# cruiseresearchgroup/ViLCo

Measured on AMD Instinct MI355X. Metric: clips/sec (fwd+bwd) MQ transformer T=2304 C=2304, higher is better.
Workload: dtype fp16 MFMA on 2-part splits of power-of-two scaled fp32 operands (22 significant bits, 3 MFMAs per product), fp32 accumulate: fp32-equivalent; weight-gradient products with contraction length >= 2048 use the leading fp16 parts only (11-bit operands, 1 MFMA; <= 3.5e-4 of the 3-MFMA gradients at this c; 1 GPU; MQ ViLCo backbone config P: T=2304 Cin=2304 D=1024 H=16 arch(2,2,5) XLNet layer text L=77x768 22 classes, train mode with the reference's dropout 0.1 / droppath 0.1 / XLNet dropout 0.1 (mq_vilco.yaml, xlnet_config_1024.json); clips_per_gpu=2, global_batch=2, parallelism=dp1

## Files before the change

include/vilco_hip.h:

```cpp
#ifndef VILCO_HIP_H
#define VILCO_HIP_H

#include <stddef.h>
#include <stdint.h>

#ifdef __cplusplus
extern "C" {
#endif

enum vilco_status {
  VILCO_OK = 0,
  VILCO_ERR_BADARG = -1,
  VILCO_ERR_UNSUPPORTED = -2,
  VILCO_ERR_LAUNCH = -3,
  VILCO_ERR_WORKSPACE = -4
};

const char* vilco_status_str(int status);
const char* vilco_version(void);
size_t vilco_abi_sizeof(const char* struct_name);

enum { VILCO_ACT_NONE = 0, VILCO_ACT_RELU = 1, VILCO_ACT_GELU = 2 };
enum { VILCO_TAP_NONE = 0, VILCO_TAP_A = 1, VILCO_TAP_B = 2 };

typedef struct vilco_gemm_desc {
  const float* A;
  const float* B;
  float* C;
  int32_t M, N, K;
  int32_t a_kcontig;
  int32_t b_kcontig;
  int64_t lda, ldb, ldc;
  int32_t batch_outer, batch_inner;
  int64_t sAo, sAi, sBo, sBi, sCo, sCi;
  int32_t tap_operand, tapC, tapT;
  int32_t precision;
  float alpha, beta;
  const float* bias;
  float* preact;
  int32_t act;
  const int32_t* row_len;
  int32_t rowT;
  const float* colscale;
  const float* residual;
  int32_t res_masked;
  void* workspace;
  size_t workspace_bytes;
  const void* a_planes;
  const void* b_planes;
  int32_t band, bandT;
  float drop_p;
  uint32_t drop_seed;
  float* amax_out;
  const float* a_amax; int32_t a_namax;
  const float* b_amax; int32_t b_namax;
  int32_t a_planes_seq, b_planes_seq;
  const float* row_mask;
} vilco_gemm_desc;

size_t vilco_gemm_workspace(const vilco_gemm_desc* d);
int vilco_gemm(const vilco_gemm_desc* d, void* stream);
int vilco_gemm_group(const vilco_gemm_desc* descs, int32_t n, void* stream);
size_t vilco_gemm_group_workspace(const vilco_gemm_desc* d, int32_t n);
int vilco_gemm_set_group_dw(int32_t on);
int32_t vilco_gemm_group_dw(void);

int vilco_gemm_force(int32_t bm, int32_t ks);
int vilco_gemm_set_skinny(int32_t on);
int64_t vilco_gemm_config_gen(void);
int32_t vilco_gemm_amax_parts(const vilco_gemm_desc* desc);
int vilco_gemm_profile_begin(void);
int vilco_gemm_profile_end(double* kernel_ms, int64_t* launches);
int64_t vilco_gemm_profile_records(int64_t* desc, double* ms, int64_t cap);

size_t vilco_pack_bytes(int64_t rows, int64_t cols, int32_t precision);
int vilco_pack(const float* src, int64_t rows, int64_t cols, int64_t ld, int32_t precision, void* planes,
               size_t planes_bytes, void* stream);
typedef struct vilco_pack_item {
  const float* src;
  int64_t rows, cols, ld;
  void* planes;
  size_t planes_bytes;
  int32_t nbatch;
  int64_t batch_stride;
  int32_t relshift;
  const float* amax;
  int32_t namax;
  int32_t seq_len;
} vilco_pack_item;
size_t vilco_pack_item_bytes(const vilco_pack_item* item, int32_t precision);
int vilco_pack_many(const vilco_pack_item* items, int32_t n, int32_t precision, void* stream);

typedef struct vilco_ln_fwd_desc {
  const float* x;
  const float* gamma;
  const float* beta;
  float* y;
  float* mean;
  float* rstd;
  int64_t rows;
  int32_t C;
  float eps;
  int32_t relu;
  float* amax_parts;
  int32_t* n_parts;
  void* planes;
  size_t planes_bytes;
  int32_t seq_len;
  const float* row_mask;
  int64_t mask_rows;
} vilco_ln_fwd_desc;
size_t vilco_layernorm_planes_bytes(int64_t rows, int32_t C, int32_t seq_len);
int vilco_layernorm_fwd(const vilco_ln_fwd_desc* d, void* stream);

typedef struct vilco_ln_bwd_desc {
// ... 441 lines not shown
```

vilco_amd/_lib.py:

```python
import ctypes as C
import os

_HERE = os.path.dirname(os.path.abspath(__file__))
if __package__:
    from . import switches
else:
    import importlib.util
    _spec = importlib.util.spec_from_file_location("vilco_switches", os.path.join(_HERE, "switches.py"))
    switches = importlib.util.module_from_spec(_spec)
    _spec.loader.exec_module(switches)
LIB_PATH = switches.text("VILCO_HIP_LIB") or os.path.join(_HERE, "libvilco_hip.so")

ACT_NONE, ACT_RELU, ACT_GELU = 0, 1, 2
TAP_NONE, TAP_A, TAP_B = 0, 1, 2

c_fp = C.c_void_p
i32, i64, f32, sz = C.c_int32, C.c_int64, C.c_float, C.c_size_t


class GemmDesc(C.Structure):
    _cname_ = "vilco_gemm_desc"
    _fields_ = [
        ("A", c_fp), ("B", c_fp), ("C", c_fp),
        ("M", i32), ("N", i32), ("K", i32),
# ... 109 lines not shown


class DistillDesc(C.Structure):
    _cname_ = "vilco_distill_desc"
    _fields_ = [("logits", c_fp), ("targets", c_fp), ("level_row", c_fp), ("level_T", c_fp), ("level_dev", c_fp),
                ("B", i32), ("R", i32), ("C", i32), ("L", i32), ("clip", i32), ("ldt", i32), ("n_known", i32), ("mode", i32),
                ("scale", f32)]


class DerDesc(C.Structure):
    _cname_ = "vilco_der_desc"
    _fields_ = [("logits", c_fp), ("level_row", c_fp), ("level_T", c_fp), ("level_dev", c_fp), ("level_len", c_fp),
                ("der_tab", c_fp), ("B", i32), ("R", i32), ("C", i32), ("L", i32), ("alpha", C.c_double)]


class PodDesc(C.Structure):
    _cname_ = "vilco_pod_desc"
    _fields_ = [("feats", c_fp), ("level_T", c_fp), ("level_len", c_fp), ("pod_tab", c_fp), ("B", i32), ("C", i32), ("L", i32),
                ("reserved", i32), ("scale", C.c_double)]


class BicCorrectDesc(C.Structure):
    _cname_ = "vilco_bic_correct_desc"
    _fields_ = [("x", c_fp), ("y", c_fp), ("splits", c_fp), ("table", c_fp), ("rows", i64), ("C", i32), ("S", i32),
                ("ldx", i32), ("ldy", i32), ("n_layers", i32)]


class PromptDesc(C.Structure):
    _cname_ = "vilco_prompt_desc"
    _fields_ = [("x", c_fp), ("prompt", c_fp), ("key", c_fp), ("cls", c_fp), ("idx_in", c_fp),
                ("B", i32), ("L", i32), ("C", i32), ("P", i32), ("len", i32), ("k", i32), ("key_mode", i32), ("vote", i32),
                ("idx", c_fp), ("sim", c_fp), ("pn", c_fp), ("xn", c_fp), ("selkey", c_fp), ("prompted", c_fp),
                ("reduce_sim", c_fp), ("workspace", c_fp), ("workspace_bytes", sz)]


class CodaDesc(C.Structure):
    _cname_ = "vilco_coda_desc"
    _fields_ = [("x", c_fp), ("prompt", c_fp), ("key", c_fp), ("attn", c_fp),
                ("B", i32), ("L", i32), ("C", i32), ("M", i32), ("len", i32), ("s", i32), ("f", i32), ("want_ortho", i32),
                ("alpha", c_fp), ("prompted", c_fp), ("ortho", c_fp), ("workspace", c_fp), ("workspace_bytes", sz)]


SIGNATURES = {
    "vilco_status_str": (C.c_char_p, [C.c_int]),
    "vilco_version": (C.c_char_p, []),
    "vilco_abi_sizeof": (sz, [C.c_char_p]),
    "vilco_defer_set": (C.c_int, [i32]),
    "vilco_defer_pending": (i64, []),
    "vilco_defer_flush": (C.c_int, [c_fp]),
    "vilco_gemm_workspace": (sz, [C.POINTER(GemmDesc)]),
    "vilco_gemm": (C.c_int, [C.POINTER(GemmDesc), c_fp]),
    "vilco_gemm_group": (C.c_int, [C.POINTER(GemmDesc), i32, c_fp]),
    "vilco_gemm_group_workspace": (sz, [C.POINTER(GemmDesc), i32]),
    "vilco_gemm_set_group_dw": (C.c_int, [i32]),
    "vilco_gemm_group_dw": (i32, []),
    "vilco_gemm_amax_parts": (i32, [C.POINTER(GemmDesc)]),
    "vilco_gemm_force": (C.c_int, [i32, i32]),
    "vilco_gemm_set_skinny": (C.c_int, [i32]),
    "vilco_gemm_config_gen": (i64, []),
    "vilco_gemm_profile_begin": (C.c_int, []),
    "vilco_gemm_profile_end": (C.c_int, [C.POINTER(C.c_double), C.POINTER(C.c_int64)]),
    "vilco_gemm_profile_records": (C.c_int64, [C.POINTER(C.c_int64), C.POINTER(C.c_double), C.c_int64]),
    "vilco_pack_bytes": (sz, [i64, i64, i32]),
    "vilco_pack_item_bytes": (sz, [C.POINTER(PackItem), i32]),
    "vilco_pack": (C.c_int, [c_fp, i64, i64, i64, i32, c_fp, sz, c_fp]),
    "vilco_pack_many": (C.c_int, [C.POINTER(PackItem), i32, i32, c_fp]),
    "vilco_layernorm_fwd": (C.c_int, [C.POINTER(LnFwdDesc), c_fp]),
    "vilco_layernorm_planes_bytes": (sz, [i64, i32, i32]),
    "vilco_layernorm_bwd_workspace": (sz, [i64, i32]),
    "vilco_layernorm_bwd": (C.c_int, [C.POINTER(LnBwdDesc), c_fp]),
    "vilco_dwconv3_fwd": (C.c_int, [c_fp, c_fp, c_fp, c_fp, i32, i32, i32, i32, c_fp]),
    "vilco_dwconv3_bwd_workspace": (sz, [i32, i32, i32, i32]),
    "vilco_dwconv3_bwd": (C.c_int, [c_fp, c_fp, c_fp, c_fp, c_fp, c_fp, i32, i32, i32, i32, c_fp, sz, c_fp]),
    "vilco_maxpool3s2_fwd": (C.c_int, [c_fp, c_fp, c_fp, i32, i32, i32, c_fp]),
    "vilco_maxpool3s2_bwd": (C.c_int, [c_fp, c_fp, c_fp, c_fp, i32, i32, i32, c_fp]),
    "vilco_softmax_fwd": (C.c_int, [c_fp, c_fp, i32, i32, i32, i32, i32, c_fp]),
    "vilco_softmax_bwd": (C.c_int, [c_fp, c_fp, i32, i32, i32, i32, c_fp]),
    "vilco_relshift_add": (C.c_int, [c_fp, c_fp, f32, i32, i32, i32, c_fp]),
    "vilco_relshift_bwd": (C.c_int, [c_fp, c_fp, f32, i32, i32, i32, c_fp]),
    "vilco_attn_supported": (C.c_int, [i32]),
    "vilco_attn_fwd_workspace": (sz, [i32, i32, i32, i32, i32, i32]),
    "vilco_attn_amax_parts": (i32, [i32, i32, i32, i32, i32, i32, i32, f32, i32]),
    "vilco_attn_fwd": (C.c_int, [C.POINTER(AttnDesc), c_fp]),
    "vilco_attn_planes_supported": (i32, [i32, i32, i32, i32, i32, i32, f32]),
    "vilco_attn_bwd_workspace": (sz, [i32, i32, i32, i32, i32, i32]),
    "vilco_attn_bwd": (C.c_int, [C.POINTER(AttnDesc), c_fp]),
    "vilco_attn_dsplanes_bytes": (sz, [i32, i32, i32]),
    "vilco_xl_scores_workspace": (sz, [i32, i32, i32, i32]),
    "vilco_xl_scores": (C.c_int, [c_fp, c_fp, c_fp, i32, i32, i32, i32, i32, i32, c_fp, sz, c_fp]),
    "vilco_decode_workspace": (sz, [i32, i32]),
    "vilco_decode": (C.c_int, [c_fp, c_fp, c_fp, c_fp, c_fp, i32, i32, i32, f32, f32, c_fp, c_fp, c_fp, c_fp, c_fp, sz, c_fp]),
    "vilco_scale_add_fwd": (C.c_int, [c_fp, c_fp, c_fp, c_fp, c_fp, c_fp, i32, i32, i32, i32, c_fp]),
    "vilco_colsum_workspace": (sz, [i64, i32]),
    "vilco_scale_add_bwd": (C.c_int, [C.POINTER(ScaleAddBwdDesc), c_fp]),
    "vilco_dropout": (C.c_int, [c_fp, c_fp, i64, f32, C.c_uint32, C.c_uint64, c_fp]),
    "vilco_attn_dropout_mask": (C.c_int, [c_fp, i64, i32, f32, C.c_uint32, c_fp]),
    "vilco_seed_word_set": (C.c_int, [C.c_uint32, c_fp]),
    "vilco_seed_word_bump": (C.c_int, [c_fp]),
    "vilco_seed_word_get": (C.c_int, [C.POINTER(C.c_uint32)]),
    "vilco_axpby": (C.c_int, [c_fp, c_fp, c_fp, f32, f32, i64, c_fp]),
    "vilco_act_bwd": (C.c_int, [C.POINTER(ActBwdDesc), c_fp]),
    "vilco_act_bwd_planes_bytes": (sz, [i64, i32, i32]),
    "vilco_colsum": (C.c_int, [c_fp, c_fp, i64, i32, c_fp, sz, c_fp]),
    "vilco_mask_rows": (C.c_int, [c_fp, c_fp, i32, i32, i32, c_fp]),
    "vilco_add_pe": (C.c_int, [c_fp, c_fp, c_fp, c_fp, i32, i32, i32, c_fp]),
    "vilco_transpose2d": (C.c_int, [c_fp, c_fp, i32, i32, i32, c_fp]),
# ... 112 lines not shown
```

vilco_amd/csrc/gemm.hip:

```cpp
#include <algorithm>
#include <climits>
#include <cstdlib>
#include <type_traits>
#include <utility>
#include <vector>
#include "common.h"
#include "pack.h"

namespace {

constexpr int BN = 128, BK = 32;
constexpr int EPI_LD = 68;

__device__ __forceinline__ int swz(int row) { return (4 - ((row >> 2) & 3)) & 3; }
__device__ __forceinline__ int lds_off(int row, int chunk) { return row * 32 + ((chunk ^ swz(row)) << 3); }

struct Epi {
  float alpha, beta;
  const float* bias;
  float* preact;
  int act;
  const int* row_len;
  int rowT;
  const float* colscale;
// ... 802 lines not shown
#pragma unroll
          for (int j = 0; j < 4; ++j) acc[i][j] = mma<true>(fa[u][0][i], fb[u][1][j], acc[i][j]);
#pragma unroll
        for (int i = 0; i < MB; ++i)
#pragma unroll
          for (int j = 0; j < 4; ++j) acc[i][j] = mma<true>(fa[u][1][i], fb[u][0][j], acc[i][j]);
      }
    }
  }

  float* mine = part + wave * (BMS * SK_LD);
#pragma unroll
  for (int i = 0; i < MB; ++i)
#pragma unroll
    for (int j = 0; j < 4; ++j)
#pragma unroll
      for (int rr = 0; rr < 4; ++rr) mine[(16 * i + (lane >> 4) * 4 + rr) * SK_LD + 16 * j + r16] = acc[i][j][rr];
  __syncthreads();
  const float inv = g.inv_a[0] * g.inv_b[0];
  float am = 0.f;
#pragma unroll 1
  for (int q = tid; q < BMS * 16; q += 512) {
    const int row = q >> 4, c4 = (q & 15) * 4;
    const float* src = part + row * SK_LD + c4;
    f32x4 v = *reinterpret_cast<const f32x4*>(src);
#pragma unroll
    for (int w = 1; w < 8; ++w) v += *reinterpret_cast<const f32x4*>(src + w * (BMS * SK_LD));
    v *= inv;
    const int m = m0 + row, n = n0 + c4;
    if (m >= g.M || n >= g.N) continue;
    const long idx = (long)m * g.ldc + n;
    bool valid = g.e.row_len ? (m % g.e.rowT) < g.e.row_len[m / g.e.rowT] : true;
    if (g.e.row_mask) valid = valid && g.e.row_mask[m] != 0.f;
    if (g.vec_out) am = fmaxf(am, store_out4(g, idx, n, v, valid));
    else
#pragma unroll 1
      for (int e = 0; e < 4; ++e) if (n + e < g.N) am = fmaxf(am, store_out(g, idx + e, n + e, v[e], valid));
  }
  if (g.amax_out) {
    am = wave_max(am);
    __syncthreads();
    if (lane == 0) part[wave] = am;
    __syncthreads();
    if (tid == 0) {
      float m = part[0];
#pragma unroll
      for (int w = 1; w < 8; ++w) m = fmaxf(m, part[w]);
      g.amax_out[blockIdx.x] = m;
    }
  }
}

template <bool VEC>
__global__ __launch_bounds__(256) void splitk_reduce_kernel(GArgs g, int nz) {
  constexpr int V = VEC ? 4 : 1;
  const int NV = g.N / V;
  const long per = (long)g.M * NV;
  const long total = per * nz;
  float am = 0.f;
  for (long i = (long)blockIdx.x * blockDim.x + threadIdx.x; i < total; i += (long)gridDim.x * blockDim.x) {
    const int z = (int)(i / per);
    const long mn = i % per;
    const int m = (int)(mn / NV), n = (int)(mn % NV) * V;
    const int zo = z / g.batch_inner, zi = z % g.batch_inner;
    const long idx = zo * g.sCo + zi * g.sCi + (long)m * g.ldc + n;
    bool valid = true;
    if (g.e.row_len) valid = (m % g.e.rowT) < g.e.row_len[m / g.e.rowT];
    if (g.e.row_mask) valid = valid && g.e.row_mask[m] != 0.f;
    if (VEC) {
      f32x4 s = {0.f, 0.f, 0.f, 0.f};
      int k = 0;
      for (; k + 4 <= g.ksplit; k += 4) {
        f32x4 v[4];
#pragma unroll
        for (int u = 0; u < 4; ++u) v[u] = *reinterpret_cast<const f32x4*>(g.c + (long)(k + u) * g.split_stride + idx);
#pragma unroll
        for (int u = 0; u < 4; ++u) s += v[u];
      }
      if (k + 2 <= g.ksplit) {
        const f32x4 v0 = *reinterpret_cast<const f32x4*>(g.c + (long)k * g.split_stride + idx);
        const f32x4 v1 = *reinterpret_cast<const f32x4*>(g.c + (long)(k + 1) * g.split_stride + idx);
        s += v0; s += v1;
        k += 2;
      }
      if (k < g.ksplit) s += *reinterpret_cast<const f32x4*>(g.c + (long)k * g.split_stride + idx);
      am = fmaxf(am, store_out4(g, idx, n, s, valid));
    } else {
      float s = 0.f;
      for (int k = 0; k < g.ksplit; ++k) s += g.c[(long)k * g.split_stride + idx];
      am = fmaxf(am, store_out(g, idx, n, s, valid));
    }
  }
  if (g.amax_out) {
    __shared__ float red[4];
    am = wave_max(am);
    if ((threadIdx.x & 63) == 0) red[threadIdx.x >> 6] = am;
    __syncthreads();
    if (threadIdx.x == 0) g.amax_out[blockIdx.x] = fmaxf(fmaxf(red[0], red[1]), fmaxf(red[2], red[3]));
  }
}

inline long align_up(long x, long a) { return (x + a - 1) / a * a; }
constexpr long SCALE_BYTES = 2 * AMAX_MAX_BLOCKS * 4 + 256;
constexpr long PACK_HDR = VILCO_PACK_HDR;

struct Config {
  const bool km = vilco_env_int("VILCO_GEMM_KM", 1, INT_MIN) != 0;
  const bool k2 = vilco_env_flag("VILCO_GEMM_K2", true);
  const bool sub192 = vilco_env_flag("VILCO_GEMM_SUB192", true);
  const bool dw_tall = vilco_env_flag("VILCO_GEMM_DW_TALL", true);
  const bool tapkm = vilco_env_flag("VILCO_CONV_DW_KM", true);
  const bool group = vilco_env_flag("VILCO_GEMM_GROUP", true);
  const int skinny_max_rows = vilco_env_int("VILCO_GEMM_SKINNY_M", 640, 1);
  const int skinny_bm16_rows = vilco_env_int("VILCO_GEMM_SKINNY_BM16", 640, 0);
  const int skinny_max_k = vilco_env_int("VILCO_GEMM_SKINNY_K", 768, 1);
  bool skinny = vilco_env_flag("VILCO_GEMM_SKINNY", true);
  bool group_dw = vilco_env_flag("VILCO_GEMM_GROUP_DW", true);
  int force_bm = vilco_env_int("VILCO_GEMM_BM", 0, INT_MIN), force_ks = vilco_env_int("VILCO_GEMM_KS", 0, INT_MIN);
};
inline Config& config() { static Config c; return c; }
inline int parts_of_precision(int precision, bool pack_abi = false) {
  if (precision == 1) return 1;
  if (precision == 0 || precision == 3) return 2;
  return (precision == 4 && !pack_abi) ? 2 : 3;
}

inline long natural_image_elems(long rows, long cols) { return align_up(rows, 32) * align_up(cols, 32); }
inline long seq_image_elems(long nseq, long T, long cols) { return align_up(vilco_tap_plane_rows(nseq, T) * cols, 8); }

struct Side {
  bool tr, km;
  int tap, out_rows;
  int nbo, nbi;
  long pack_batch;
  long bytes;
  long batch, plane;
};
struct Layout { int NP, Kp; bool tapkm; Side a, b; };

bool tapkm_layout(const vilco_gemm_desc* d, Layout& L) {
  if (!(config().km && config().tapkm && (d->tapC % 8) == 0 && (d->M % 8) == 0 && d->tapT > 0 && (d->K % d->tapT) == 0 &&
        d->batch_outer == 1 && d->batch_inner == 1))
    return false;
  Side &a = L.a, &b = L.b;
  const long nseq = d->K / d->tapT;
  L.Kp = (int)align_up(nseq * (d->tapT + 2) - 1, 32);
  a.tap = b.tap = 1; a.tr = b.tr = false; a.km = b.km = true;
  a.out_rows = L.Kp + 1 + 32; b.out_rows = L.Kp + 3 + 32;
  a.pack_batch = (long)a.out_rows * d->M; b.pack_batch = (long)b.out_rows * d->tapC;
  return true;
}
long prepacked_a(const vilco_gemm_desc* d, const Layout& L) {
  if (L.a.tap != 1) return natural_image_elems(d->M, L.Kp);
  return L.tapkm ? seq_image_elems(d->K / d->tapT, d->tapT, d->M) : seq_image_elems(d->M / d->tapT, d->tapT, d->tapC);
}
long prepacked_b(const vilco_gemm_desc* d, const Layout& L) {
  return L.tapkm ? seq_image_elems(d->K / d->tapT, d->tapT, d->tapC) : natural_image_elems(d->N, L.Kp);
}
void finish_side(const vilco_gemm_desc* d, int NP, Side& s, long so, long si, long image) {
  s.nbo = (so && d->batch_outer > 1) ? d->batch_outer : 1;
  s.nbi = (si && d->batch_inner > 1) ? d->batch_inner : 1;
  s.pack_batch = align_up(s.pack_batch, 8);
  s.bytes = align_up(s.pack_batch * s.nbo * s.nbi * NP * 2, 256);
  s.batch = image >= 0 ? image : s.pack_batch;
  s.plane = s.batch * s.nbo * s.nbi;
}
Layout operand_layout(const vilco_gemm_desc* d, bool a_prepacked, bool b_prepacked) {
  Layout L;
// ... 489 lines not shown
    if (it.planes_bytes < vilco_pack_item_bytes(&it, precision)) return VILCO_ERR_WORKSPACE;
    const long cols = item_cols(it);
    const long rows32 = align_up(it.rows, 32), cols32 = align_up(cols, 32);
    float* hdr = reinterpret_cast<float*>(it.planes);
    PackArgs& pa = pk.a[i];
    pa.src = it.src; pa.dst = reinterpret_cast<__bf16*>(reinterpret_cast<unsigned char*>(it.planes) + PACK_HDR);
    pa.ld = it.ld; pa.rows = (int)it.rows; pa.K = (int)cols; pa.Kp = (int)cols32;
    pa.plane_stride = rows32 * cols32 * nbatch; pa.batch_stride = rows32 * cols32; pa.nbi = nbatch;
    pa.so = 0; pa.si = nbatch > 1 ? it.batch_stride : 0;
    pa.tap = it.relshift ? 4 : 0; pa.tapC = it.relshift ? (int)it.cols : 1; pa.tapT = 1; pa.out_rows = (int)rows32;
    pa.vec = vilco_aligned(it.src, 16) && (it.ld % 4) == 0 && (it.batch_stride % 4) == 0;
    if (it.seq_len > 0) {
      if (it.relshift || nbatch != 1 || (it.cols % 8) != 0 || (it.rows % it.seq_len) != 0) return VILCO_ERR_UNSUPPORTED;
      const long tr = vilco_tap_plane_rows(it.rows / it.seq_len, it.seq_len);
      pa.tap = 1; pa.tapC = (int)it.cols; pa.tapT = it.seq_len; pa.out_rows = (int)tr;
      pa.plane_stride = align_up(tr * it.cols, 8); pa.batch_stride = pa.plane_stride;
    }
    pa.amax = nullptr; pa.namax = 0; pa.inv_scale = hdr + AMAX_MAX_BLOCKS;
    if (precision == 3) {
      PackArgs src_view = pa;
      src_view.K = (int)it.cols; src_view.tap = 0;
      am.op[i] = amax_view(src_view, false, 1, hdr);
      pa.amax = hdr; pa.namax = am.op[i].nblocks;
      if (it.amax && it.namax > 0) { pa.amax = it.amax; pa.namax = it.namax; have_amax[i] = true; }
    }
  }
  if (precision == 3) {
    int todo = 0;
    for (int i = 0; i < n; ++i) todo += have_amax[i] ? 0 : 1;
    if (todo) {
      AmaxArgs am2;
      int k = 0;
      for (int i = 0; i < n; ++i)
        if (!have_amax[i]) am2.op[k++] = am.op[i];
      launch_amax(am2, k, s);
    }
  }
  if (n == 1 && nbatch == 1) dispatch_pack(NP, pk.a[0], false, 1, s);
  else dispatch_pack_multi(NP, pk, n, s, nbatch);
  return vilco_launch_status();
}

extern "C" int vilco_pack(const float* src, int64_t rows, int64_t cols, int64_t ld, int32_t precision, void* planes,
                          size_t planes_bytes, void* stream) {
  const vilco_pack_item it = {src, rows, cols, ld, planes, planes_bytes, 1, 0, 0, nullptr, 0};
  return vilco_pack_many(&it, 1, precision, stream);
}

extern "C" size_t vilco_gemm_workspace(const vilco_gemm_desc* d) {
  if (!d || d->M <= 0 || d->N <= 0 || d->K < 0) return 512;
  return workspace_need(make_plan(d));
}

static void splitk_finish(const vilco_gemm_desc* d, const Prepared& pr) {
  const GArgs& g = pr.g;
  if (vilco_defer_active() && pr.nz == 1 && d->alpha == 1.f && d->beta == 0.f && !d->bias &&
      !d->preact && d->act == VILCO_ACT_NONE && !d->row_len && !d->row_mask && !d->colscale && !d->residual && d->drop_p == 0.f &&
      !d->amax_out) {
    vilco_defer_push_sk(g.c, g.cfinal, g.split_stride, g.ldc, d->M, d->N, pr.p.ksplit);
    return;
  }
  const dim3 blocks((int)splitk_blocks(d));
  if (g.vec_out) hipLaunchKernelGGL(splitk_reduce_kernel<true>, blocks, dim3(256), 0, pr.s, g, pr.nz);
  else hipLaunchKernelGGL(splitk_reduce_kernel<false>, blocks, dim3(256), 0, pr.s, g, pr.nz);
}

extern "C" int vilco_gemm(const vilco_gemm_desc* d, void* stream) {
  Prepared pr;
  const int rc = gemm_prepare(d, stream, pr);
  if (rc != VILCO_OK || pr.empty) return rc;
  const Plan& p = pr.p;
  {
    ProfScope timed(pr.s, ProfRec{{d->M, d->N, d->K, pr.nz, p.BM, p.ksplit, d->precision, p.a.km, p.b.km, p.a.tap | (p.b.tap << 4)}});
    launch_plan(p, pr.g, dim3(pr.g.ntiles, p.ksplit, pr.nz), pr.s);
  }
  if (p.ksplit > 1) splitk_finish(d, pr);
  return vilco_launch_status();
}

static bool group_dw_member(const vilco_gemm_desc& d, const vilco_gemm_desc& d0) {
  return d.a_planes && d.b_planes && d.precision == 4 && d.batch_outer == 1 && d.batch_inner == 1 && d.tap_operand == VILCO_TAP_NONE &&
         d.band == 0 && d.M == d0.M && d.N == d0.N && d.K == d0.K && d.ldc == d0.ldc && d.a_kcontig == d0.a_kcontig &&
         d.b_kcontig == d0.b_kcontig && d.M > 0 && d.N > 0 && d.alpha == 1.f && d.beta == 0.f && !d.bias && !d.preact &&
         d.act == VILCO_ACT_NONE && !d.row_len && !d.row_mask && !d.colscale && !d.residual && d.drop_p == 0.f && !d.amax_out;
}
static bool group_dw_allowed() {
  const Config& c = config();
  return c.group && c.group_dw && c.km && c.k2 && c.force_bm == 0 && c.force_ks < 1;
}

static inline int group_launch_size(int n) { const int l = (n + GROUP_MAX - 1) / GROUP_MAX; return l ? (n + l - 1) / l : 0; }

extern "C" size_t vilco_gemm_group_workspace(const vilco_gemm_desc* d, int32_t n) {
  if (!d || d->M <= 0 || d->N <= 0 || d->K < 0) return 512;
  const Plan p = make_plan(d);
  size_t need = workspace_need(p);
  if (n >= 2 && d->precision == 4 && p.kern == Kern::PP_K2 && group_dw_allowed())
    for (int m = group_launch_size(n); m >= 2 && m >= group_launch_size(n) - 1; --m) {
      Tiling t;
      Plan pg = p;
      if (plan_group_dw(d, p, p.Kp, m, t)) { pg.part_bytes = t.part_bytes; need = std::max(need, workspace_need(pg)); }
    }
  return need;
}

static bool gemm_group_dw(const vilco_gemm_desc* descs, int n, void* stream, int& rc) {
  if (n < 2 || !group_dw_allowed()) return false;
  std::vector<Prepared> prs(n);
  Tiling t;
  for (int i = 0; i < n; ++i) {
    const vilco_gemm_desc& d = descs[i];
// ... 1 lines not shown
    if (!group_dw_member(d, descs[0]) || gemm_prepare(&d, stream, pr) != VILCO_OK || pr.p.kern != Kern::PP_K2) return false;
    if (i == 0 && !plan_group_dw(&d, pr.p, pr.p.Kp, n, t)) return false;
    Plan pg = pr.p;
    pg.part_bytes = t.part_bytes;
    if (d.workspace_bytes < workspace_need(pg) || pr.g.vec_out != prs[0].g.vec_out || pr.p.a.km != prs[0].p.a.km || pr.p.b.km != prs[0].p.b.km)
      return false;
    static_cast<Tiling&>(pr.p) = t;
    GArgs& g = pr.g;
    g.ntiles = g.tiles_n * ((d.M + t.BM - 1) / t.BM);
    g.ksplit = t.ksplit; g.kchunk = t.kchunk; g.split_stride = t.split_stride;
    g.c = t.ksplit > 1 ? pr.parts : d.C;
  }
  GArgsG gg;
  gg.g = prs[0].g;
  gg.n = n;
  for (int i = 0; i < n; ++i) gg.e[i] = GroupEnt{prs[i].g.a.p, prs[i].g.b.p, prs[i].g.c, prs[i].g.cfinal, prs[i].g.inv_a, prs[i].g.inv_b};
  for (int i = n; i < GROUP_MAX; ++i) gg.e[i] = gg.e[0];
  hipStream_t s = prs[0].s;
  const Plan& p0 = prs[0].p;
  {
    ProfScope timed(s, ProfRec{{descs[0].M, descs[0].N, descs[0].K, n, t.BM, t.ksplit, 4, p0.a.km, p0.b.km, 0x100}});
    const dim3 grid(gg.g.ntiles * n, t.ksplit, 1);
    with_bm<256, 128>(t.BM, [&](auto R) {
      constexpr int BM = decltype(R)::value;
      with_km(p0.a.km, p0.b.km, [&](auto A, auto B) {
        constexpr bool AKM = decltype(A)::value, BKM = decltype(B)::value;
        launch_gemm<&gemm_pp_group_kernel<BM, AKM, BKM>>(pp_lds<BM, 2, AKM, BKM>(), grid, s, gg);
      });
    });
  }
  if (t.ksplit > 1)
    for (int i = 0; i < n; ++i) splitk_finish(&descs[i], prs[i]);
  rc = vilco_launch_status();
  return true;
}

extern "C" int vilco_gemm_group(const vilco_gemm_desc* descs, int32_t n, void* stream) {
  if (!descs || n < 1) return VILCO_ERR_BADARG;
  if (descs[0].precision == 4) {
    const int launches = (n + GROUP_MAX - 1) / GROUP_MAX;
    for (int l = 0, i0 = 0; l < launches; ++l) {
      const int m = group_launch_size(n) - (l >= launches - (group_launch_size(n) * launches - n) ? 1 : 0);
      int rc = VILCO_OK;
      if (!gemm_group_dw(descs + i0, m, stream, rc))
        for (int i = i0; i < i0 + m && rc == VILCO_OK; ++i) rc = vilco_gemm(&descs[i], stream);
      if (rc != VILCO_OK) return rc;
      i0 += m;
    }
    return VILCO_OK;
  }
  if (n > 4) return VILCO_ERR_BADARG;
  hipStream_t s = reinterpret_cast<hipStream_t>(stream);
  GArgsN gg;
  Plan p0;
  bool ok = config().group && n >= 2;
  for (int i = 0; ok && i < n; ++i) {
    const vilco_gemm_desc& d = descs[i];
    Prepared pr;
    ok = d.a_planes && d.b_planes && d.precision == 3 && d.batch_outer == 1 && d.batch_inner == 1 && d.tap_operand == VILCO_TAP_NONE &&
         d.band == 0 && d.M == descs[0].M && d.N == descs[0].N && d.K == descs[0].K && d.a_kcontig == descs[0].a_kcontig &&
         d.b_kcontig == descs[0].b_kcontig && d.M > 0 && d.N > 0 && gemm_prepare(&d, stream, pr) == VILCO_OK &&
         pr.p.kern == Kern::GL && pr.p.ksplit == 1 && (i == 0 || (pr.p.BM == p0.BM && pr.p.a.km == p0.a.km && pr.p.b.km == p0.b.km));
    if (!ok) break;
    gg.g[i] = pr.g;
    if (i == 0) p0 = pr.p;
  }
  if (!ok) {
    for (int i = 0; i < n; ++i) {
      const int rc = vilco_gemm(&descs[i], stream);
      if (rc != VILCO_OK) return rc;
    }
    return VILCO_OK;
  }
  {
    ProfScope timed(s, ProfRec{{descs[0].M, descs[0].N, descs[0].K, n, p0.BM, 1, 3, p0.a.km, p0.b.km, 0x100}});
    const dim3 grid(gg.g[0].ntiles, 1, n);
    with_bm<192, 128>(p0.BM, [&](auto R) {
      constexpr int BM = decltype(R)::value;
      with_km(p0.a.km, p0.b.km, [&](auto A, auto B) {
        launch_gemm<&gemm_gl_group_kernel<BM, decltype(A)::value, decltype(B)::value>>(gl_lds<BM>(), grid, s, gg);
      });
    });
  }
  return vilco_launch_status();
}

static int64_t g_config_gen = 0;
extern "C" int64_t vilco_gemm_config_gen(void) { return g_config_gen; }

extern "C" int vilco_gemm_set_skinny(int32_t on) {
  config().skinny = on != 0;
  ++g_config_gen;
  return VILCO_OK;
}

extern "C" int vilco_gemm_set_group_dw(int32_t on) {
  config().group_dw = on != 0;
  ++g_config_gen;
  return VILCO_OK;
}
extern "C" int32_t vilco_gemm_group_dw(void) { return config().group_dw ? 1 : 0; }

extern "C" int vilco_gemm_force(int32_t bm, int32_t ks) {
  if (bm < 0 || ks < 0) return VILCO_ERR_BADARG;
  config().force_bm = bm; config().force_ks = ks;
  ++g_config_gen;
  return VILCO_OK;
}
```

vilco_amd/ops.py:

```python
import ctypes as C
import math

import torch

from . import _lib, switches
from ._lib import ACT_GELU, ACT_NONE, ACT_RELU, TAP_A, TAP_B, TAP_NONE, GemmDesc

_PRECISIONS = {"split": 0, 0: 0, "bf16": 1, 1: 1, "split3": 2, "fp32": 2, 2: 2, "f16x2": 3, 3: 3}
DEFAULT_PRECISION = _PRECISIONS[switches.text("VILCO_PRECISION")]
_precision = DEFAULT_PRECISION


_DW = {"f16x1": 4, "f16x2": None}
dw_precision = _DW[switches.text("VILCO_DW_PRECISION")]
DW_FAST_MIN_K = 2048


def _dw_prec(prec, K=0):
    return dw_precision if (dw_precision is not None and prec == 3 and K >= DW_FAST_MIN_K) else prec


def set_precision(p=None):
    global _precision
    _precision = DEFAULT_PRECISION if p is None else _PRECISIONS[p]
# ... 488 lines not shown
    if parts is not None:
        it.amax, it.namax = parts.data_ptr(), n
    if nbytes is None:
        nbytes = _lib.load().vilco_pack_item_bytes(C.byref(it), prec)
    buf = torch.empty(nbytes, dtype=torch.uint8, device=x.device)
    it.planes, it.planes_bytes = buf.data_ptr(), nbytes
    return buf


def pack(x, rows, cols, precision=None):
    lib = _lib.load()
    prec = _precision if precision is None else int(precision)
    buf = _planes_of(x, "nat", (rows, cols), prec)
    if buf is not None:
        return buf
    nbytes = lib.vilco_pack_bytes(int(rows), int(cols), prec)
    if prec != 3 or _amax_of(x)[0] is None:
        buf = torch.empty(nbytes, dtype=torch.uint8, device=x.device)
        _lib.check(lib.vilco_pack(x.data_ptr(), int(rows), int(cols), int(cols), prec, buf.data_ptr(), nbytes, _stream()))
    else:
        it = _lib.PackItem()
        buf = _pack_item(it, x, rows, cols, prec, nbytes=nbytes)
        _lib.check(lib.vilco_pack_many(C.byref(it), 1, prec, _stream()))
    return _remember_planes(x, "nat", (rows, cols), prec, buf)


def pack_tap(x, precision=None):
    prec = _precision if precision is None else int(precision)
    buf = _planes_of(x, "seq", x.shape, prec)
    if buf is not None:
        return buf
    B, T, Cn = x.shape
    it = _lib.PackItem()
    buf = _pack_item(it, x, B * T, Cn, prec, seq_len=T)
    _lib.check(_lib.load().vilco_pack_many(C.byref(it), 1, prec, _stream()))
    return _remember_planes(x, "seq", x.shape, prec, buf)


def pack_many(items, precision=None, nbatch=1, relshift=False):
    prec = _precision if precision is None else int(precision)
    arr = (_lib.PackItem * len(items))()
    bufs = [_pack_item(it, x, rows, cols, prec, nbatch, relshift) for it, (x, rows, cols) in zip(arr, items)]
    _lib.check(_lib.load().vilco_pack_many(arr, len(items), prec, _stream()))
    return bufs


pack_group_enabled = switches.on("VILCO_PACK_GROUP")
ln_bwd_amax = switches.on("VILCO_LN_BWD_AMAX")
conv_dz_planes = switches.on("VILCO_CONV_DZ_PLANES")


def pack_group(xs, rows, cols, precision=None):
    prec = _precision if precision is None else int(precision)
    n = len(xs)
    fresh = all(_planes_of(x, "nat", (rows, cols), prec, any_stream=True) is None for x in xs)
    if (not pack_group_enabled or not (2 <= n <= 4) or not fresh or len({x.data_ptr() for x in xs}) != n
            or any(not x.is_contiguous() for x in xs)):
        return [pack(x, rows, cols, precision) for x in xs]
    bufs = pack_many([(x, rows, cols) for x in xs], precision=prec)
    return [_remember_planes(x, "nat", (rows, cols), prec, buf) for x, buf in zip(xs, bufs)]


_reuse_packs = switches.on("VILCO_PACK_REUSE")
conv_tap_planes = switches.on("VILCO_CONV_TAP_PLANES") and switches.on("VILCO_CONV_DW_KM")

_weight_cache = switches.on("VILCO_WEIGHT_CACHE")
_weight_gen = [0]


def weights_changed():
    _weight_gen[0] += 1


def _cached(w, tag, build):
    if not _weight_cache:
        return build()
    owner = w._base if w._base is not None else w
    if owner.requires_grad and not owner.is_leaf:
        return build()
    store = owner.__dict__.setdefault("_vilco_cache", {})
    key = (tag, w.data_ptr(), tuple(w.shape), _precision)
    ver = (owner._version, _weight_gen[0])
    ent = store.get(key)
    if ent is not None and ent[0] == ver:
        return ent[1]
    val = build()
    store[key] = (ver, val)
    return val


def forget_weight_planes(params):
    for p in params:
        p.__dict__.pop("_vilco_cache", None)


def tag_weight_amax(p, parts, n):
    p._vilco_wamax = (parts, int(n), p._version, _weight_gen[0])


def _weight_amax(w):
    owner = w._base if w._base is not None else w
    tag = getattr(owner, "_vilco_wamax", None)
    if (tag is None or not produce_amax or _precision != 3 or tag[2] != owner._version or tag[3] != _weight_gen[0]
            or w.numel() != owner.numel()):
        return None, 0
    return tag[0], tag[1]
# ... 1985 lines not shown
```

vilco_amd/switches.py:

```python
import os
from collections import namedtuple

Switch = namedtuple("Switch", "env default readers key meaning")

KEYED = "keyed"
VIA_SET = "ops.set_precision moves ops._precision, which is keyed"
ONCE = "read once per process"
GEN = "read once per process; its setter bumps vilco_gemm_config_gen(), which is part of ops.arithmetic_key()"
BUILT = "read at construction and fixed in the object"
INFERENCE = "inference only"
HOST = "host scheduling only"
PENDING = "unkeyed as before although a flip changes what LayerNorm / attention forward record: to be keyed in a follow-up"

TABLE = (
    Switch("VILCO_PRECISION", "f16x2", ("ops.DEFAULT_PRECISION",), VIA_SET, "operand format of the matrix products"),
    Switch("VILCO_DW_PRECISION", "f16x1", ("ops.dw_precision",), KEYED, "long weight-gradient products read the leading fp16 part only"),
    Switch("VILCO_GRAPH_STREAMS", "text,heads", ("ops._FORKS",), KEYED, "chains forked onto side streams inside a captured step"),
    Switch("VILCO_DW_FORK_ROWS", "0", ("ops._dw_fork_rows",), KEYED, "with 'dw' forked: only products over at most this many token rows"),
    Switch("VILCO_DEFER_FINISH", "1", ("ops.defer_finish",), KEYED, "second stages of backward's reductions issued together at its end"),
    Switch("VILCO_RANGE_CHECK", "0", ("ops.range_check",), KEYED, "warn | auto: measure the row spread of every Linear backward's dZ"),
    Switch("VILCO_PRODUCER_AMAX", "1", ("ops.produce_amax",), KEYED, "producers leave max|x| partials for the operand packs"),
    Switch("VILCO_PACK_CACHE", "1", ("ops._pack_cache",), PENDING, "an activation's operand planes are remembered on the tensor"),
    Switch("VILCO_PACK_GROUP", "1", ("ops.pack_group_enabled",), KEYED, "the packs of a grouped q / k / v projection as one launch"),
    Switch("VILCO_LN_BWD_AMAX", "1", ("ops.ln_bwd_amax",), KEYED, "LayerNorm backward leaves max|dx| partials"),
    Switch("VILCO_CONV_DZ_PLANES", "1", ("ops.conv_dz_planes",), KEYED, "masked k=3 convs: dZ's operand image from the mask kernel"),
    Switch("VILCO_PACK_REUSE", "1", ("ops._reuse_packs",), KEYED, "one pack of a tensor serves forward, dX and dW"),
    Switch("VILCO_CONV_TAP_PLANES", "1", ("ops.conv_tap_planes",), KEYED, "k=3 convs: x and dZ packed once each for all three products"),
    Switch("VILCO_CONV_DW_KM", "1", ("ops.conv_tap_planes", "gemm.hip"), KEYED, "... and their weight gradient reads those images k-major"),
    Switch("VILCO_WEIGHT_CACHE", "1", ("ops._weight_cache",), KEYED, "weight operand planes kept per parameter version"),
    Switch("VILCO_PRODUCER_PLANES", "1", ("ops.producer_planes",), KEYED, "activation backward writes dz as operand planes"),
    Switch("VILCO_LN_PLANES", "1", ("ops.ln_planes",), KEYED, "LayerNorm forward writes its output as operand planes"),
    Switch("VILCO_ATTN_PLANES", "1", ("ops.attn_planes",), KEYED, "hd = 64 attention forward writes its output as operand planes"),
    Switch("VILCO_LINEAR_GROUP", "1", ("ops.linear_group_enabled",), KEYED, "q / k / v projections as one grouped GEMM launch"),
    Switch(None, "1", ("ops.use_flash",), KEYED, "fused attention kernels (off: materialised scores)"),
    Switch("VILCO_FOLD_SKIP", "1", ("ops.fold_skip_grads",), KEYED, "skip gradients added inside the LayerNorm backward kernel"),
    Switch("VILCO_XL_DS_PLANES", "1", ("ops.xl_ds_planes",), KEYED, "XLNet backward: dS as operand planes from the dQ kernel"),
    Switch("VILCO_XL_SCORES", "1", ("ops.xl_scores_kernel",), KEYED, "XLNet forward: position scores by their own kernel"),
    Switch("VILCO_FUSED_PROMPT", "1", ("ops.fused_prompt",), KEYED, "L2P prompt pool: match, vote and prepend kernels"),
    Switch("VILCO_QKV_PRE", "1", ("ops.use_qkv_pre",), KEYED, "fused ln1 -> depthwise convs -> LayerNorms kernel in MaskedMHCA"),
    Switch("VILCO_HIP_LIB", "", ("_lib.LIB_PATH",), ONCE, "library to load instead of vilco_amd/libvilco_hip.so"),
    Switch("VILCO_DP_REPLAY_SYNC", "1", ("graph._DP_REPLAY_SYNC",), HOST, "data-parallel replays wait for the graph before a CPU-side exchange"),
    Switch("VILCO_GRAPH_OWN_STREAM", "1", ("graph._OWN_STREAM",), HOST, "replays leave the default stream for a created one"),
    Switch("VILCO_GRAPH_SHARED_STREAM", "1", ("graph._SHARED_STREAM",), HOST, "... shared by every GraphedStep of the process"),
    Switch("VILCO_DP_SEGMENTS", "1", ("graph._DP_SEGMENTS",), BUILT, "data-parallel backward captured as one graph per stage"),
    Switch("VILCO_DP_GRAPH_COMM", "0", ("graph.GraphedStep.comm_in_graph",), BUILT, "1: the all-reduces captured inside the graph"),
    Switch("VILCO_OPT_AMAX", "1", ("utils.train_utils.OPT_AMAX",), ONCE, "the optimizer update leaves max|w| per chunk for the weight packs"),
    Switch("VILCO_CA_WIDE", "qkv,core,proj", ("modeling.blocks.ChannelAttention.WIDE_PARTS",), ONCE, "channel-attention parts run in bf16 x3"),
    Switch("VILCO_XLNET_CONFIG_DIR", "", ("modeling.backbones._find_xlnet_config",), BUILT, "where xlnet_config_<D>.json is looked for first"),
    Switch("VILCO_HEAD_ROWMASK", "1", ("modeling.meta_archs._HEAD_ROWMASK",), ONCE, "the heads' validity mask applied in the GEMM epilogue"),
    Switch("VILCO_LEVEL_CAT", "1", ("PtTransformer.level_cat",), BUILT, "both heads run over all pyramid levels at once"),
    Switch("VILCO_SYNC_FREE_LOSS", "1", ("PtTransformer.sync_free_loss",), BUILT, "dense, host-sync-free evaluation of the losses"),
    Switch("VILCO_FUSED_LOSS", "1", ("PtTransformer.fused_loss",), BUILT, "ops.mq_loss kernels (0: tensor expressions)"),
    Switch("VILCO_FUSED_SSL", "1", ("PtTransformer.fused_ssl",), BUILT, "ops.ssl_pool / ssl_nce kernels (0: tensor expressions)"),
    Switch("VILCO_DEVICE_DECODE", "1", ("PtTransformer.inference_single_video",), INFERENCE, "vilco_decode (0: the tensor-expression decode)"),
    Switch("VILCO_ATTN_FAST", "1", ("attn.hip",), ONCE, "hd = 64 attention fast-path kernels"),
    Switch("VILCO_ATTN_XL_FAST", "1", ("attn.hip",), ONCE, "XLNet's relative attention on the hd = 64 fast-path kernels"),
    Switch("VILCO_LAB_ATTN_LDS", "", ("attn.hip",), ONCE, "-DVILCO_LAB_ATTN builds only: the attention kernels' LDS request"),
    Switch("VILCO_GEMM_KM", "1", ("gemm.hip",), ONCE, "transposed operands read k-major from natural-layout planes"),
    Switch("VILCO_GEMM_K2", "1", ("gemm.hip",), ONCE, "single-part products cover two K-steps per barrier interval"),
    Switch("VILCO_GEMM_SUB192", "1", ("gemm.hip",), ONCE, "the two sub-round 192-row plans"),
    Switch("VILCO_GEMM_DW_TALL", "1", ("gemm.hip",), ONCE, "single-part weight-gradient products planned on 192- / 256-row tiles"),
    Switch("VILCO_GEMM_GROUP", "1", ("gemm.hip",), ONCE, "grouped GEMM launches"),
    Switch("VILCO_GEMM_GROUP_DW", "1", ("gemm.hip",), GEN, "initial vilco_gemm_set_group_dw: a backward's equal single-part weight gradients as one launch"),
    Switch("VILCO_GEMM_SKINNY", "1", ("gemm.hip",), ONCE, "initial vilco_gemm_set_skinny: skinny NT products on small workgroups"),
    Switch("VILCO_GEMM_SKINNY_M", "640", ("gemm.hip",), ONCE, "largest M of a skinny product"),
    Switch("VILCO_GEMM_SKINNY_BM16", "640", ("gemm.hip",), ONCE, "largest M on 16-row workgroups"),
    Switch("VILCO_GEMM_SKINNY_K", "768", ("gemm.hip",), ONCE, "largest K of a skinny product"),
    Switch("VILCO_GEMM_BM", "0", ("gemm.hip",), ONCE, "initial vilco_gemm_force: tile height"),
    Switch("VILCO_GEMM_KS", "0", ("gemm.hip",), ONCE, "initial vilco_gemm_force: split-K count"),
    Switch("VILCO_ACT_BWD_VEC", "1", ("eltwise.hip",), ONCE, "four channels per thread in the activation-backward kernel"),
    Switch("VILCO_QKV_TB", "0", ("qkvpre.hip",), ONCE, "forced tokens per workgroup of the three-pass q/k/v pre-projection"),
    Switch("VILCO_QKV_RING", "-1", ("qkvpre.hip",), ONCE, "1 / 0: the ring form of the q/k/v pre-projection always / never"),
    Switch("VILCO_PACK_CAP", "768", ("pack.h",), ONCE, "workgroup cap of the natural-layout pack kernel"),
    Switch("VILCO_SOFTNMS_LEGACY", "0", ("nms.hip",), ONCE, "initial vilco_nms_set_kernel: 1 = one pass per pick only"),
    Switch("VILCO_SOFTNMS_REG", "1", ("nms.hip",), ONCE, "initial vilco_nms_set_kernel: 0 = nothing faster than the row-strided kernel"),
)

_DEFAULT = {s.env: s.default for s in TABLE if s.env is not None}
KEYED_OPS = tuple(dict.fromkeys(r[4:] for s in TABLE if s.key == KEYED for r in s.readers if r.startswith("ops.")))


def text(env):
    return os.environ.get(env, _DEFAULT[env])


def on(env):
    return text(env) != "0"


def number(env):
    return int(text(env))
```

Baseline: 102.1 clips/s.

## Allow split-K plans in grouped GEMM launches with a grouped reduce kernel

New measurement: 102.9 clips/s, median of 6. About the same (+0.7%).

```diff
diff --git a/include/vilco_hip.h b/include/vilco_hip.h
--- a/include/vilco_hip.h
+++ b/include/vilco_hip.h
@@ -61,6 +61,8 @@
 size_t vilco_gemm_workspace(const vilco_gemm_desc* d);
 int vilco_gemm(const vilco_gemm_desc* d, void* stream);
 int vilco_gemm_group(const vilco_gemm_desc* descs, int32_t n, void* stream);
+int vilco_gemm_set_group(int32_t on);
+int32_t vilco_gemm_group_on(void);
 size_t vilco_gemm_group_workspace(const vilco_gemm_desc* d, int32_t n);
 int vilco_gemm_set_group_dw(int32_t on);
 int32_t vilco_gemm_group_dw(void);
diff --git a/vilco_amd/_lib.py b/vilco_amd/_lib.py
--- a/vilco_amd/_lib.py
+++ b/vilco_amd/_lib.py
@@ -185,6 +185,8 @@
     "vilco_gemm": (C.c_int, [C.POINTER(GemmDesc), c_fp]),
     "vilco_gemm_group": (C.c_int, [C.POINTER(GemmDesc), i32, c_fp]),
     "vilco_gemm_group_workspace": (sz, [C.POINTER(GemmDesc), i32]),
+    "vilco_gemm_set_group": (C.c_int, [i32]),
+    "vilco_gemm_group_on": (i32, []),
     "vilco_gemm_set_group_dw": (C.c_int, [i32]),
     "vilco_gemm_group_dw": (i32, []),
     "vilco_gemm_amax_parts": (i32, [C.POINTER(GemmDesc)]),
diff --git a/vilco_amd/csrc/gemm.hip b/vilco_amd/csrc/gemm.hip
--- a/vilco_amd/csrc/gemm.hip
+++ b/vilco_amd/csrc/gemm.hip
@@ -878,7 +878,7 @@
 }
 
 template <bool VEC>
-__global__ __launch_bounds__(256) void splitk_reduce_kernel(GArgs g, int nz) {
+__device__ __forceinline__ void splitk_reduce_body(const GArgs& g, int nz) {
   constexpr int V = VEC ? 4 : 1;
   const int NV = g.N / V;
   const long per = (long)g.M * NV;
@@ -925,6 +925,14 @@
     if (threadIdx.x == 0) g.amax_out[blockIdx.x] = fmaxf(fmaxf(red[0], red[1]), fmaxf(red[2], red[3]));
   }
 }
+template <bool VEC>
+__global__ __launch_bounds__(256) void splitk_reduce_kernel(GArgs g, int nz) {
+  splitk_reduce_body<VEC>(g, nz);
+}
+template <bool VEC>
+__global__ __launch_bounds__(256) void splitk_reduce_group_kernel(GArgsN gg) {
+  splitk_reduce_body<VEC>(gg.g[blockIdx.y], 1);
+}
 
 inline long align_up(long x, long a) { return (x + a - 1) / a * a; }
 constexpr long SCALE_BYTES = 2 * AMAX_MAX_BLOCKS * 4 + 256;
@@ -936,10 +944,11 @@
   const bool sub192 = vilco_env_flag("VILCO_GEMM_SUB192", true);
   const bool dw_tall = vilco_env_flag("VILCO_GEMM_DW_TALL", true);
   const bool tapkm = vilco_env_flag("VILCO_CONV_DW_KM", true);
-  const bool group = vilco_env_flag("VILCO_GEMM_GROUP", true);
   const int skinny_max_rows = vilco_env_int("VILCO_GEMM_SKINNY_M", 640, 1);
   const int skinny_bm16_rows = vilco_env_int("VILCO_GEMM_SKINNY_BM16", 640, 0);
   const int skinny_max_k = vilco_env_int("VILCO_GEMM_SKINNY_K", 768, 1);
+  const int group_split_rows = vilco_env_int("VILCO_GEMM_GROUP_SPLIT_M", 1152, 0);
+  bool group = vilco_env_flag("VILCO_GEMM_GROUP", true);
   bool skinny = vilco_env_flag("VILCO_GEMM_SKINNY", true);
   bool group_dw = vilco_env_flag("VILCO_GEMM_GROUP_DW", true);
   int force_bm = vilco_env_int("VILCO_GEMM_BM", 0, INT_MIN), force_ks = vilco_env_int("VILCO_GEMM_KS", 0, INT_MIN);
@@ -1535,11 +1544,14 @@
   return workspace_need(make_plan(d));
 }
 
+static bool splitk_deferred(const vilco_gemm_desc* d, const Prepared& pr) {
+  return vilco_defer_active() && pr.nz == 1 && d->alpha == 1.f && d->beta == 0.f && !d->bias &&
+         !d->preact && d->act == VILCO_ACT_NONE && !d->row_len && !d->row_mask && !d->colscale && !d->residual && d->drop_p == 0.f &&
+         !d->amax_out;
+}
 static void splitk_finish(const vilco_gemm_desc* d, const Prepared& pr) {
   const GArgs& g = pr.g;
-  if (vilco_defer_active() && pr.nz == 1 && d->alpha == 1.f && d->beta == 0.f && !d->bias &&
-      !d->preact && d->act == VILCO_ACT_NONE && !d->row_len && !d->row_mask && !d->colscale && !d->residual && d->drop_p == 0.f &&
-      !d->amax_out) {
+  if (splitk_deferred(d, pr)) {
     vilco_defer_push_sk(g.c, g.cfinal, g.split_stride, g.ldc, d->M, d->N, pr.p.ksplit);
     return;
   }
@@ -1647,18 +1659,26 @@
   if (n > 4) return VILCO_ERR_BADARG;
   hipStream_t s = reinterpret_cast<hipStream_t>(stream);
   GArgsN gg;
-  Plan p0;
+  Prepared prs[4];
   bool ok = config().group && n >= 2;
   for (int i = 0; ok && i < n; ++i) {
     const vilco_gemm_desc& d = descs[i];
-    Prepared pr;
+    Prepared& pr = prs[i];
+    const Plan& p0 = prs[0].p;
     ok = d.a_planes && d.b_planes && d.precision == 3 && d.batch_outer == 1 && d.batch_inner == 1 && d.tap_operand == VILCO_TAP_NONE &&
          d.band == 0 && d.M == descs[0].M && d.N == descs[0].N && d.K == descs[0].K && d.a_kcontig == descs[0].a_kcontig &&
          d.b_kcontig == descs[0].b_kcontig && d.M > 0 && d.N > 0 && gemm_prepare(&d, stream, pr) == VILCO_OK &&
-         pr.p.kern == Kern::GL && pr.p.ksplit == 1 && (i == 0 || (pr.p.BM == p0.BM && pr.p.a.km == p0.a.km && pr.p.b.km == p0.b.km));
+         pr.p.kern == Kern::GL && (pr.p.BM == p0.BM && pr.p.ksplit == p0.ksplit && pr.p.a.km == p0.a.km && pr.p.b.km == p0.b.km);
+    if (ok && pr.p.ksplit > 1) {
+      ok = d.M <= config().group_split_rows && pr.g.vec_out == prs[0].g.vec_out && !splitk_deferred(&d, pr);
+      const char* lo = reinterpret_cast<const char*>(pr.parts);
+      for (int j = 0; ok && j < i; ++j) {
+        const char* lo_j = reinterpret_cast<const char*>(prs[j].parts);
+        ok = lo + pr.p.part_bytes <= lo_j || lo_j + prs[j].p.part_bytes <= lo;
+      }
+    }
     if (!ok) break;
     gg.g[i] = pr.g;
-    if (i == 0) p0 = pr.p;
   }
   if (!ok) {
     for (int i = 0; i < n; ++i) {
@@ -1667,9 +1687,10 @@
     }
     return VILCO_OK;
   }
+  const Plan& p0 = prs[0].p;
   {
-    ProfScope timed(s, ProfRec{{descs[0].M, descs[0].N, descs[0].K, n, p0.BM, 1, 3, p0.a.km, p0.b.km, 0x100}});
-    const dim3 grid(gg.g[0].ntiles, 1, n);
+    ProfScope timed(s, ProfRec{{descs[0].M, descs[0].N, descs[0].K, n, p0.BM, p0.ksplit, 3, p0.a.km, p0.b.km, 0x100}});
+    const dim3 grid(gg.g[0].ntiles, p0.ksplit, n);
     with_bm<192, 128>(p0.BM, [&](auto R) {
       constexpr int BM = decltype(R)::value;
       with_km(p0.a.km, p0.b.km, [&](auto A, auto B) {
@@ -1677,6 +1698,11 @@
       });
     });
   }
+  if (p0.ksplit > 1) {
+    const dim3 blocks((int)splitk_blocks(&descs[0]), n);
+    if (gg.g[0].vec_out) hipLaunchKernelGGL(splitk_reduce_group_kernel<true>, blocks, dim3(256), 0, s, gg);
+    else hipLaunchKernelGGL(splitk_reduce_group_kernel<false>, blocks, dim3(256), 0, s, gg);
+  }
   return vilco_launch_status();
 }
 
@@ -1688,6 +1714,13 @@
   ++g_config_gen;
   return VILCO_OK;
 }
+
+extern "C" int vilco_gemm_set_group(int32_t on) {
+  config().group = on != 0;
+  ++g_config_gen;
+  return VILCO_OK;
+}
+extern "C" int32_t vilco_gemm_group_on(void) { return config().group ? 1 : 0; }
 
 extern "C" int vilco_gemm_set_group_dw(int32_t on) {
   config().group_dw = on != 0;
diff --git a/vilco_amd/ops.py b/vilco_amd/ops.py
--- a/vilco_amd/ops.py
+++ b/vilco_amd/ops.py
@@ -564,6 +564,12 @@
 
 def pack_group(xs, rows, cols, precision=None):
     prec = _precision if precision is None else int(precision)
+    first = {}
+    for x in xs:
+        first.setdefault(id(x), x)
+    if len(first) < len(xs):
+        bufs = dict(zip(first, pack_group(list(first.values()), rows, cols, precision)))
+        return [bufs[id(x)] for x in xs]
     n = len(xs)
     fresh = all(_planes_of(x, "nat", (rows, cols), prec, any_stream=True) is None for x in xs)
     if (not pack_group_enabled or not (2 <= n <= 4) or not fresh or len({x.data_ptr() for x in xs}) != n
diff --git a/vilco_amd/switches.py b/vilco_amd/switches.py
--- a/vilco_amd/switches.py
+++ b/vilco_amd/switches.py
@@ -60,7 +60,8 @@
     Switch("VILCO_GEMM_K2", "1", ("gemm.hip",), ONCE, "single-part products cover two K-steps per barrier interval"),
     Switch("VILCO_GEMM_SUB192", "1", ("gemm.hip",), ONCE, "the two sub-round 192-row plans"),
     Switch("VILCO_GEMM_DW_TALL", "1", ("gemm.hip",), ONCE, "single-part weight-gradient products planned on 192- / 256-row tiles"),
-    Switch("VILCO_GEMM_GROUP", "1", ("gemm.hip",), ONCE, "grouped GEMM launches"),
+    Switch("VILCO_GEMM_GROUP", "1", ("gemm.hip",), GEN, "initial vilco_gemm_set_group: grouped GEMM launches"),
+    Switch("VILCO_GEMM_GROUP_SPLIT_M", "1152", ("gemm.hip",), ONCE, "largest M of a two-part group that runs its split-K plan as one launch"),
     Switch("VILCO_GEMM_GROUP_DW", "1", ("gemm.hip",), GEN, "initial vilco_gemm_set_group_dw: a backward's equal single-part weight gradients as one launch"),
     Switch("VILCO_GEMM_SKINNY", "1", ("gemm.hip",), ONCE, "initial vilco_gemm_set_skinny: skinny NT products on small workgroups"),
     Switch("VILCO_GEMM_SKINNY_M", "640", ("gemm.hip",), ONCE, "largest M of a skinny product"),
```
